# cts198859/deeprl_network

Measured on NVIDIA H100. Metric: agent-env-steps/sec CACC Catch-up NeurComm A2C, higher is better.
Workload: dtype f32

## Files before the change

deeprl_network_b200/csrc/tc_wgrad.cu:

```cuda
#include "bwd_common.cuh"
#include "tc_row.cuh"

extern long long* g_nmarl_prof;

namespace {
using namespace tcrow;

enum { J_GATE0 = 0, J_GATE1, J_ENC_X, J_ENC_M0, J_ENC_M1, J_COUNT };
constexpr int WG_LANES = 128, WG_HALF = 64;
constexpr int WG_A_THREADS = WG_LANES, WG_THREADS = WG_A_THREADS + 2 * 128;
constexpr uint32_t WG_A_TILE = WG_LANES * 128, WG_A_SLOT = 2 * WG_A_TILE;
constexpr uint32_t WG_RING = 224 * 1024;
constexpr int WG_MAX_BARS = 32;
constexpr size_t WG_SMEM = 1024 + WG_RING + WG_MAX_BARS * 8;
static_assert(WG_SMEM <= 232448, "wgrad rings exceed the 227 KB of dynamic shared memory");
static_assert(WG_HALF == ROWS, "each MMA warpgroup covers the 64 rows of one wgmma");
constexpr int WG_REGS_A = 120, WG_REGS_MMA = 192;
static_assert(WG_A_THREADS * WG_REGS_A + 256 * WG_REGS_MMA <= WG_THREADS * 168, "setmaxnreg split exceeds the CTA's registers");
constexpr int SEG_KB = 20;

__device__ __forceinline__ void wg_depths(int N, int& S, int& A) {
  S = N >= 256 ? 2 : (N >= 192 ? 3 : (N >= 128 ? 4 : 6));
  A = (int)((WG_RING - (uint32_t)S * 256u * (uint32_t)N) / WG_A_SLOT);
  if (A > 4) A = 4;
}

struct RingPos {
  int idx = 0; uint32_t ph = 0;
  __device__ __forceinline__ void next(int n) { if (++idx == n) { idx = 0; ph ^= 1u; } }
};

struct TcWgK {
  int B, T, splits, ndp;
  const float* sv_sh; const float* sv_xin; const float* dzT; const float* dpT;
  const float* h_seq; const float* done_pre;
  float* ws;
  long long ws_off[J_COUNT];
  int jobs[J_COUNT]; int n_jobs;
  int* err;
  long long* prof;
};

struct JobDesc {
  const float* A; int F_A, a_feat0, ka_cnt, ones;
  int p_feat0, p_cnt;
  const float* BT; int tile_rows, n_row0, N;
};

__device__ __forceinline__ JobDesc job_desc(const nmarl_model& m, const TcWgK& k, int kind, int i) {
  const nmarl_agent& ag = m.agent[i];
  JobDesc d;
  d.p_feat0 = 0; d.p_cnt = 0;
  const int SD = m.s_dim, LDI = m.kx_pad + m.kp_pad + m.km_pad;
  const int Km = (m.variant == NMARL_IC3) ? NH : ag.n_nbr * NH;
  if (kind == J_GATE0 || kind == J_GATE1) {
    const int mt = kind - J_GATE0;
    d.A = k.sv_sh; d.F_A = SD + NH; d.a_feat0 = 128 * mt; d.ka_cnt = max(0, min(128, SD + NH - 128 * mt)); d.ones = 0;
    d.BT = k.dzT; d.tile_rows = 256; d.n_row0 = 0; d.N = 256;
  } else if (kind == J_ENC_X) {
    d.A = k.sv_xin; d.F_A = LDI; d.a_feat0 = 0; d.ka_cnt = ag.x_nsrc * ag.x_w; d.ones = 1;
    if (m.variant == NMARL_NC) { d.p_feat0 = m.kx_pad; d.p_cnt = ag.n_nbr * m.n_a; }
    d.BT = k.dpT; d.tile_rows = k.ndp; d.n_row0 = 0; d.N = k.ndp;
  } else {
    const int mt = kind - J_ENC_M0;
    d.A = k.sv_xin; d.F_A = LDI; d.a_feat0 = m.kx_pad + m.kp_pad + 128 * mt; d.ka_cnt = max(0, min(128, Km - 128 * mt)); d.ones = 0;
    d.BT = k.dpT; d.tile_rows = k.ndp; d.n_row0 = (m.variant == NMARL_NC) ? 128 : 64; d.N = 64;
  }
  return d;
}

template <bool RAW>
__global__ void __launch_bounds__(WG_THREADS, 1) tc_wgrad_kernel(const __grid_constant__ nmarl_model m,
                                                                 const __grid_constant__ TcWgK k) {
  extern __shared__ uint8_t smem_raw[];
  uint8_t* smem = reinterpret_cast<uint8_t*>((reinterpret_cast<uintptr_t>(smem_raw) + 1023) & ~uintptr_t(1023));

  const int sp = blockIdx.x, jslot = blockIdx.y, i = blockIdx.z;
  const int kind = k.jobs[jslot];
  const JobDesc d = job_desc(m, k, kind, i);
  const int lanes = d.ka_cnt > 0 ? d.ka_cnt + d.ones + d.p_cnt : 0;
  const int nact = (lanes + WG_HALF - 1) / WG_HALF;
  if (nact == 0) return;
  int S, AS;
  wg_depths(d.N, S, AS);
  uint8_t* bst = smem;
  uint8_t* ast = smem + (size_t)S * 256 * d.N;
  uint64_t* bars = reinterpret_cast<uint64_t*>(smem + WG_RING);
  uint64_t *b_full = bars, *b_split = b_full + S, *b_empty = b_split + S, *a_full = b_empty + S, *a_empty = a_full + AS;

  const int N_agents = m.n_agent;
  const int tid = threadIdx.x, warp = tid >> 5;
  const int bpt = k.B / 32;
  const int kb_total = k.T * bpt;
  const int per = (kb_total + k.splits - 1) / k.splits;
  const int kb0 = sp * per, kb1 = min(kb_total, kb0 + per);
  const int nkb = (d.ka_cnt > 0) ? max(0, kb1 - kb0) : 0;
  float* wsj = k.ws + k.ws_off[jslot] + ((size_t)sp * N_agents + i) * 128 * d.N;

  if (tid == 0) {
    for (int s = 0; s < S; ++s) { tc::mbar_init(&b_full[s], 1); tc::mbar_init(&b_split[s], WG_A_THREADS); tc::mbar_init(&b_empty[s], 4 * nact); }
    for (int s = 0; s < AS; ++s) { tc::mbar_init(&a_full[s], WG_A_THREADS); tc::mbar_init(&a_empty[s], 4 * nact); }
    tc::fence_barrier_init();
  }
  __syncthreads();
  const uint32_t tile_bytes = (uint32_t)d.N * 128u;

  if (warp < WG_A_THREADS / 32) {
    asm volatile("setmaxnreg.dec.sync.aligned.u32 %0;" ::"n"(WG_REGS_A));
    const int row = tid;
    const bool on = row < WG_HALF * nact;
    const int ka = row;
    const bool one = d.ones && ka == d.ka_cnt;
    const bool is_p = ka > d.ka_cnt && ka <= d.ka_cnt + d.p_cnt;
    const bool real = on && (ka < d.ka_cnt || is_p);
    const int feat = is_p ? d.p_feat0 + (ka - d.ka_cnt - 1) : d.a_feat0 + ka;
    int hs_agent = -1, hs_unit = 0;
    bool hs_mask = false;
    if (k.h_seq != nullptr && real && !is_p) {
      if ((kind == J_GATE0 || kind == J_GATE1) && feat >= m.s_dim) { hs_agent = i; hs_unit = feat - m.s_dim; hs_mask = true; }
      else if ((kind == J_ENC_M0 || kind == J_ENC_M1) && m.variant == NMARL_NC) {
        const int fm = feat - (m.kx_pad + m.kp_pad);
        hs_agent = m.agent[i].nbr[fm / NH]; hs_unit = fm % NH;
      }
    }
    auto load_x = [&](int q, float (&x)[32]) {
      const int kb = kb0 + q, t = kb / bpt, rb = kb - t * bpt;
      if (hs_agent >= 0) {
        const float* src = k.h_seq + (((size_t)t * N_agents + hs_agent) * NH + hs_unit) * k.B + rb * 32;
#pragma unroll
        for (int p = 0; p < 8; ++p) {
          const float4 v = __ldg(reinterpret_cast<const float4*>(src + 4 * p));
          x[4 * p] = v.x; x[4 * p + 1] = v.y; x[4 * p + 2] = v.z; x[4 * p + 3] = v.w;
        }
        if (hs_mask) {
          const float* dn = k.done_pre + (size_t)t * k.B + rb * 32;
#pragma unroll
          for (int p = 0; p < 8; ++p) {
            const float4 v = __ldg(reinterpret_cast<const float4*>(dn + 4 * p));
            x[4 * p] *= 1.0f - v.x; x[4 * p + 1] *= 1.0f - v.y; x[4 * p + 2] *= 1.0f - v.z; x[4 * p + 3] *= 1.0f - v.w;
          }
        }
      } else if (real) {
        const float* src = d.A + (((size_t)t * N_agents + i) * d.F_A + feat) * k.B + rb * 32;
#pragma unroll
        for (int p = 0; p < 8; ++p) {
          const float4 v = __ldcs(reinterpret_cast<const float4*>(src + 4 * p));
          x[4 * p] = v.x; x[4 * p + 1] = v.y; x[4 * p + 2] = v.z; x[4 * p + 3] = v.w;
        }
      } else {
#pragma unroll
        for (int j = 0; j < 32; ++j) x[j] = one ? 1.0f : 0.0f;
      }
    };
    float xa[32], xb[32];
    RingPos as, bs;
    auto emit_a = [&](int q, float (&x)[32]) {
      tc::mbar_wait(&a_empty[as.idx], as.ph ^ 1, k.err, 11);
      if (on) {
        uint8_t* hi = ast + (size_t)as.idx * WG_A_SLOT;
#pragma unroll
        for (int c = 0; c < 4; ++c) {
          float x8[8];
#pragma unroll
          for (int j = 0; j < 8; ++j) x8[j] = x[8 * c + j];
          tc::st_hilo8(hi, hi + WG_A_TILE, (uint32_t)row, (uint32_t)(8 * c), x8);
        }
        tc::fence_proxy_async();
      }
      tc::mbar_arrive(&a_full[as.idx]);
      as.next(AS);
      if (q + 2 < nkb) load_x(q + 2, x);
      if constexpr (RAW) {
        tc::mbar_wait(&b_full[bs.idx], bs.ph, k.err, 31);
        float4* bhi = reinterpret_cast<float4*>(bst + (size_t)bs.idx * 2 * tile_bytes);
        float4* blo = reinterpret_cast<float4*>(bst + (size_t)bs.idx * 2 * tile_bytes + tile_bytes);
        for (uint32_t e = (uint32_t)tid; e < tile_bytes / 16; e += WG_A_THREADS) {
          const float4 v = bhi[e];
          float4 h, lo4;
          tc::split_tf32(v.x, h.x, lo4.x); tc::split_tf32(v.y, h.y, lo4.y);
          tc::split_tf32(v.z, h.z, lo4.z); tc::split_tf32(v.w, h.w, lo4.w);
          bhi[e] = h;
          blo[e] = lo4;
        }
        tc::fence_proxy_async();
        tc::mbar_arrive(&b_split[bs.idx]);
        bs.next(S);
      }
    };
    if (nkb > 0) load_x(0, xa);
    if (nkb > 1) load_x(1, xb);
    for (int q = 0; q < nkb; q += 2) {
      emit_a(q, xa);
      if (q + 1 < nkb) emit_a(q + 1, xb);
    }
  } else {
    const int g = warp / 4 - 1;
    if (g >= nact) return;
    asm volatile("setmaxnreg.inc.sync.aligned.u32 %0;" ::"n"(WG_REGS_MMA));
    const int t = tid - (g + 1) * 128, w = t >> 5, l = t & 31;
    const bool issuer = g == 0 && t == 0;
    float* out = wsj + g * WG_HALF + 16 * w + (l >> 2);
    long long* prof = (issuer && k.prof != nullptr && sp == 0 && i == 0) ? k.prof + (size_t)jslot * 1024 : nullptr;
    if (prof) { prof[0] = clock64(); prof[3] = kind | (d.N << 8); }
    auto fetch = [&](int q, int st) {
      const int kb = kb0 + q;
      const int tt = kb / bpt, rb = kb - tt * bpt;
      const size_t pair = (size_t)(2 * d.tile_rows * 128);
      const size_t off = RAW ? (size_t)tt * N_agents * bpt * pair + ((size_t)i * bpt + rb) * (pair / 2)
                             : (((size_t)tt * N_agents + i) * bpt + rb) * pair;
      const uint8_t* tile = reinterpret_cast<const uint8_t*>(d.BT) + off;
      uint8_t* dst = bst + (size_t)st * 2 * tile_bytes;
      tc::mbar_arrive_expect_tx(&b_full[st], RAW ? tile_bytes : 2 * tile_bytes);
      tc::bulk_g2s(dst, tile + (size_t)d.n_row0 * 128, tile_bytes, &b_full[st]);
      if (!RAW) tc::bulk_g2s(dst + tile_bytes, tile + (size_t)(d.tile_rows + d.n_row0) * 128, tile_bytes, &b_full[st]);
    };
    if (issuer)
      for (int q = 0; q < S && q < nkb; ++q) fetch(q, q);
    float acc[128];
#pragma unroll
    for (int j = 0; j < 128; ++j) acc[j] = 0.f;
    auto drain = [&](bool rmw) {
#pragma unroll
      for (int j = 0; j < 32; ++j) {
        if (8 * j < d.N) {
          const int n = 8 * j + 2 * (l & 3);
#pragma unroll
          for (int e = 0; e < 4; ++e) {
            float* o = out + (size_t)(n + (e & 1)) * 128 + 8 * (e >> 1);
            *o = rmw ? *o + acc[4 * j + e] : acc[4 * j + e];
          }
        }
      }
    };
    RingPos as, bs;
    for (int q = 0; q < nkb; ++q) {
      const bool seg_first = (q % SEG_KB) == 0;
      uint8_t* b = bst + (size_t)bs.idx * 2 * tile_bytes;
      if constexpr (RAW) tc::mbar_wait(&b_split[bs.idx], bs.ph, k.err, 33);
      else tc::mbar_wait(&b_full[bs.idx], bs.ph, k.err, 31);
      if (prof && q < 300) prof[4 + 3 * q] = clock64();
      tc::mbar_wait(&a_full[as.idx], as.ph, k.err, 32);
      if (prof && q < 300) prof[5 + 3 * q] = clock64();
      uint8_t* a = ast + (size_t)as.idx * WG_A_SLOT + g * (WG_A_TILE / 2);
      tc::wgmma_fence();
      tc::wgmma_kblock_3x(d.N, acc, tc::smem_desc_sw128(a), tc::smem_desc_sw128(a + WG_A_TILE), tc::smem_desc_sw128(b),
                          tc::smem_desc_sw128(b + tile_bytes), 4, seg_first);
      tc::wgmma_commit();
      tc::wgmma_wait_all();
      if (prof && q < 300) prof[6 + 3 * q] = clock64();
      if (l == 0) { tc::mbar_arrive(&a_empty[as.idx]); tc::mbar_arrive(&b_empty[bs.idx]); }
      if (issuer && q + S < nkb) {
        tc::mbar_wait(&b_empty[bs.idx], bs.ph, k.err, 34);
        fetch(q + S, bs.idx);
      }
      as.next(AS); bs.next(S);
      if ((q + 1) % SEG_KB == 0 || q + 1 == nkb) drain(q >= SEG_KB);
    }
    if (nkb == 0) drain(false);
    if (prof) { prof[1] = min(nkb, 300); prof[2] = clock64(); }
  }
}

__global__ void __launch_bounds__(256) tc_wgrad_reduce_kernel(const __grid_constant__ nmarl_model m, const __grid_constant__ TcWgK k,
                                                             float* __restrict__ grads) {
  const int jslot = blockIdx.y, i = blockIdx.z, kind = k.jobs[jslot];
  const JobDesc d = job_desc(m, k, kind, i);
  const nmarl_agent& ag = m.agent[i];
  const int lanes = d.ka_cnt + (d.ones ? 1 : 0) + d.p_cnt;
  const int total = 128 * d.N;
  for (int e = blockIdx.x * blockDim.x + threadIdx.x; e < total; e += gridDim.x * blockDim.x) {
    const int ln = e & 127, n = e >> 7;
    if (ln >= lanes) continue;
    float s = 0.f;
    for (int sp = 0; sp < k.splits; ++sp) s += k.ws[k.ws_off[jslot] + (((size_t)sp * m.n_agent + i) * d.N + n) * 128 + ln];
    if (kind == J_GATE0 || kind == J_GATE1) grads[ag.o_wxh + (size_t)(128 * (kind - J_GATE0) + ln) * NG + n] = s;
    else if (kind == J_ENC_X) {
      if (ln < d.ka_cnt) { if (n < NH) grads[ag.o_w_ob + ln * NH + n] = s; }
      else if (ln > d.ka_cnt) { if (n >= NH && n < 2 * NH) grads[ag.o_w_fp + (ln - d.ka_cnt - 1) * NH + n - NH] = s; }
      else if (n < NH) grads[ag.o_b_ob + n] = s;
      else if (m.variant == NMARL_NC && n < 2 * NH) grads[ag.o_b_fp + n - NH] = s;
      else if (ag.o_b_msg >= 0) grads[ag.o_b_msg + n - ((m.variant == NMARL_NC) ? 2 * NH : NH)] = s;
    } else grads[ag.o_w_msg + (size_t)(128 * (kind - J_ENC_M0) + ln) * NH + n] = s;
  }
}

__global__ void __launch_bounds__(256) gate_bias_reduce_kernel(const __grid_constant__ nmarl_model m, const float* __restrict__ part,
                                                              int tiles, int T, float* __restrict__ grads) {
  __shared__ float red[8][32];
  const int c = threadIdx.x & 31, p = threadIdx.x >> 5, col = blockIdx.x * 32 + c, i = blockIdx.y;
  const int n = T * tiles;
  float s = 0.f;
  for (int e = p; e < n; e += 8) {
    const int t = e / tiles, tile = e - t * tiles;
    s += part[(((size_t)t * m.n_agent + i) * tiles + tile) * NG + col];
  }
  red[p][c] = s;
  __syncthreads();
  if (p == 0) {
    float tsum = 0.f;
    for (int w = 0; w < 8; ++w) tsum += red[w][c];
    grads[m.agent[i].o_b + col] = tsum;
  }
}

NMARL_PARAMS_FIT(nmarl_model, TcWgK);
NMARL_PARAMS_FIT(nmarl_model, TcWgK, float*);
NMARL_PARAMS_FIT(nmarl_model, const float*, int, int, float*);

int job_list(const nmarl_model* m, int* jobs) {
  int n = 0;
  jobs[n++] = J_GATE0;
  if (m->s_dim + NH > 128) jobs[n++] = J_GATE1;
  jobs[n++] = J_ENC_X;
  if (m->variant != NMARL_IA2C) {
    jobs[n++] = J_ENC_M0;
    if (m->km_pad > 128) jobs[n++] = J_ENC_M1;
  }
  return n;
}
int job_N(const nmarl_model* m, int kind) {
  if (kind == J_GATE0 || kind == J_GATE1) return 256;
  if (kind == J_ENC_X) return nmarl_tc_ndp(m);
  return 64;
}

}

int nmarl_tc_ndp(const nmarl_model* m) { return m->variant == NMARL_NC ? 192 : (m->variant == NMARL_IA2C ? 64 : 128); }

int nmarl_tc_wgrad_splits(int n_agent) {
  int s = 33;
  while (4 * s * n_agent > 132 * 8 && s > 1) s = (s + 1) / 2;
  return s;
}

int64_t nmarl_tc_wgrad_ws_floats(const nmarl_model* m) {
  int jobs[J_COUNT];
  const int nj = job_list(m, jobs);
  int64_t tot = 0;
  for (int j = 0; j < nj; ++j) tot += (int64_t)nmarl_tc_wgrad_splits(m->n_agent) * m->n_agent * 128 * job_N(m, jobs[j]);
  return tot;
}

int nmarl_tc_launch_wgrads(const nmarl_model* m, int B, int T, const float* sv_sh, const float* sv_xin, const float* dzT,
                           const float* dpT, const float* sv_dz, float* ws, float* grads, int* err, cudaStream_t st,
                           cudaStream_t st_bias, bool raw_tiles, void** ev_wgrad, const float* h_seq, const float* done_pre) {
  TcWgK k{};
  k.B = B; k.T = T; k.splits = nmarl_tc_wgrad_splits(m->n_agent); k.ndp = nmarl_tc_ndp(m);
  k.sv_sh = sv_sh; k.sv_xin = sv_xin; k.dzT = dzT; k.dpT = dpT; k.ws = ws; k.err = err;
  k.h_seq = h_seq; k.done_pre = done_pre; k.prof = g_nmarl_prof;
  k.n_jobs = job_list(m, k.jobs);
  long long off = 0;
  for (int j = 0; j < k.n_jobs; ++j) { k.ws_off[j] = off; off += (long long)k.splits * m->n_agent * 128 * job_N(m, k.jobs[j]); }
  static bool configured = false;
  if (!configured) {
    NMARL_CUDA(cudaFuncSetAttribute(tc_wgrad_kernel<false>, cudaFuncAttributeMaxDynamicSharedMemorySize, (int)WG_SMEM));
    NMARL_CUDA(cudaFuncSetAttribute(tc_wgrad_kernel<true>, cudaFuncAttributeMaxDynamicSharedMemorySize, (int)WG_SMEM));
    configured = true;
  }
  gate_bias_reduce_kernel<<<dim3(NG / 32, m->n_agent), 256, 0, st_bias>>>(*m, sv_dz, B / 32, T, grads);
  NMARL_LAUNCH_CHECK();
  if (ev_wgrad) NMARL_CUDA(cudaEventRecord((cudaEvent_t)ev_wgrad[0], st));
  const dim3 grid(k.splits, k.n_jobs, m->n_agent);
  if (raw_tiles) tc_wgrad_kernel<true><<<grid, WG_THREADS, WG_SMEM, st>>>(*m, k);
  else tc_wgrad_kernel<false><<<grid, WG_THREADS, WG_SMEM, st>>>(*m, k);
  NMARL_LAUNCH_CHECK();
  if (ev_wgrad) NMARL_CUDA(cudaEventRecord((cudaEvent_t)ev_wgrad[1], st));
  NMARL_DBG_SYNC(st, "tc_wgrad_kernel");
  tc_wgrad_reduce_kernel<<<dim3(64, k.n_jobs, m->n_agent), 256, 0, st>>>(*m, k, grads);
  NMARL_LAUNCH_CHECK();
  NMARL_DBG_SYNC(st, "tc_wgrad_reduce");
  return 0;
}
```

Measured before the change: 52.87 million.

## Stage wgrad A-operand loads through cp.async landing buffers and specialize MMA loop on N

The A-producer warps now prefetch their activation rows with cp.async into a swizzled, double-buffered shared-memory landing zone one k-block ahead. The done mask also goes through this path. This replaces the register-held two-deep ldg pipeline and the emit_a lambda. The MMA consumer loop is templated on N (64/128/192/256) so the wgmma k-block and the drain are compile-time unrolled. Ring depths are retuned: N=192 now uses 2 B stages, and the A depth is reduced to make room for the landing buffers. The split and A-store ordering is also merged under one fence. Together this is meant to free producer registers and hide global latency, at the cost of extra shared memory and fewer A/B ring stages.

```diff
diff --git a/deeprl_network_b200/csrc/tc_wgrad.cu b/deeprl_network_b200/csrc/tc_wgrad.cu
--- a/deeprl_network_b200/csrc/tc_wgrad.cu
+++ b/deeprl_network_b200/csrc/tc_wgrad.cu
@@ -1,5 +1,6 @@
 #include "bwd_common.cuh"
 #include "tc_row.cuh"
+#include <type_traits>
 
 extern long long* g_nmarl_prof;
 
@@ -12,7 +13,8 @@
 constexpr uint32_t WG_A_TILE = WG_LANES * 128, WG_A_SLOT = 2 * WG_A_TILE;
 constexpr uint32_t WG_RING = 224 * 1024;
 constexpr int WG_MAX_BARS = 32;
-constexpr size_t WG_SMEM = 1024 + WG_RING + WG_MAX_BARS * 8;
+constexpr uint32_t WG_LAND = WG_LANES * 128;
+constexpr size_t WG_SMEM = 1024 + WG_RING + WG_MAX_BARS * 8 + 4 * 2 * 128;
 static_assert(WG_SMEM <= 232448, "wgrad rings exceed the 227 KB of dynamic shared memory");
 static_assert(WG_HALF == ROWS, "each MMA warpgroup covers the 64 rows of one wgmma");
 constexpr int WG_REGS_A = 120, WG_REGS_MMA = 192;
@@ -20,10 +22,17 @@
 constexpr int SEG_KB = 20;
 
 __device__ __forceinline__ void wg_depths(int N, int& S, int& A) {
-  S = N >= 256 ? 2 : (N >= 192 ? 3 : (N >= 128 ? 4 : 6));
-  A = (int)((WG_RING - (uint32_t)S * 256u * (uint32_t)N) / WG_A_SLOT);
+  S = N >= 192 ? 2 : (N >= 128 ? 4 : 6);
+  A = (int)((WG_RING - (uint32_t)S * 256u * (uint32_t)N - 2 * WG_LAND) / WG_A_SLOT);
   if (A > 4) A = 4;
 }
+
+__device__ __forceinline__ void cp_async16(void* smem_dst, const void* gsrc) {
+  asm volatile("cp.async.cg.shared.global [%0], [%1], 16;" ::"r"(tc::smem_u32(smem_dst)), "l"(gsrc) : "memory");
+}
+__device__ __forceinline__ void cp_async_commit() { asm volatile("cp.async.commit_group;" ::: "memory"); }
+template <int N>
+__device__ __forceinline__ void cp_async_wait() { asm volatile("cp.async.wait_group %0;" ::"n"(N) : "memory"); }
 
 struct RingPos {
   int idx = 0; uint32_t ph = 0;
@@ -123,57 +132,59 @@
         hs_agent = m.agent[i].nbr[fm / NH]; hs_unit = fm % NH;
       }
     }
-    auto load_x = [&](int q, float (&x)[32]) {
-      const int kb = kb0 + q, t = kb / bpt, rb = kb - t * bpt;
-      if (hs_agent >= 0) {
-        const float* src = k.h_seq + (((size_t)t * N_agents + hs_agent) * NH + hs_unit) * k.B + rb * 32;
-#pragma unroll
-        for (int p = 0; p < 8; ++p) {
-          const float4 v = __ldg(reinterpret_cast<const float4*>(src + 4 * p));
-          x[4 * p] = v.x; x[4 * p + 1] = v.y; x[4 * p + 2] = v.z; x[4 * p + 3] = v.w;
+    const bool gate_hs = k.h_seq != nullptr && (kind == J_GATE0 || kind == J_GATE1);
+    const int lane = tid & 31;
+    uint8_t* land = ast + (size_t)AS * WG_A_SLOT;
+    float* dn_sm = reinterpret_cast<float*>(smem + WG_RING + WG_MAX_BARS * 8) + warp * 2 * 32;
+    auto issue = [&](int q) {
+      if (q < nkb) {
+        const int kb = kb0 + q, t = kb / bpt, rb = kb - t * bpt;
+        const float* src = hs_agent >= 0 ? k.h_seq + (((size_t)t * N_agents + hs_agent) * NH + hs_unit) * k.B + rb * 32
+                         : real ? d.A + (((size_t)t * N_agents + i) * d.F_A + feat) * k.B + rb * 32 : nullptr;
+        if (src != nullptr) {
+          uint8_t* dst = land + (size_t)(q & 1) * WG_LAND + (size_t)row * 128;
+#pragma unroll
+          for (int c = 0; c < 8; ++c) cp_async16(dst + (((c ^ row) & 7) << 4), src + 4 * c);
+        }
+        if (gate_hs) {
+          __syncwarp();
+          if (lane < 8) cp_async16(dn_sm + (q & 1) * 32 + 4 * lane, k.done_pre + (size_t)t * k.B + rb * 32 + 4 * lane);
+        }
+      }
+      cp_async_commit();
+    };
+    auto read_x = [&](int q, float (&x)[32]) {
+      cp_async_wait<1>();
+      if (gate_hs) __syncwarp();
+      if (hs_agent >= 0 || real) {
+        const uint8_t* src = land + (size_t)(q & 1) * WG_LAND + (size_t)row * 128;
+#pragma unroll
+        for (int c = 0; c < 8; ++c) {
+          const float4 v = *reinterpret_cast<const float4*>(src + (((c ^ row) & 7) << 4));
+          x[4 * c] = v.x; x[4 * c + 1] = v.y; x[4 * c + 2] = v.z; x[4 * c + 3] = v.w;
         }
         if (hs_mask) {
-          const float* dn = k.done_pre + (size_t)t * k.B + rb * 32;
+          const float4* dn = reinterpret_cast<const float4*>(dn_sm + (q & 1) * 32);
 #pragma unroll
           for (int p = 0; p < 8; ++p) {
-            const float4 v = __ldg(reinterpret_cast<const float4*>(dn + 4 * p));
+            const float4 v = dn[p];
             x[4 * p] *= 1.0f - v.x; x[4 * p + 1] *= 1.0f - v.y; x[4 * p + 2] *= 1.0f - v.z; x[4 * p + 3] *= 1.0f - v.w;
           }
         }
-      } else if (real) {
-        const float* src = d.A + (((size_t)t * N_agents + i) * d.F_A + feat) * k.B + rb * 32;
-#pragma unroll
-        for (int p = 0; p < 8; ++p) {
-          const float4 v = __ldcs(reinterpret_cast<const float4*>(src + 4 * p));
-          x[4 * p] = v.x; x[4 * p + 1] = v.y; x[4 * p + 2] = v.z; x[4 * p + 3] = v.w;
-        }
       } else {
 #pragma unroll
         for (int j = 0; j < 32; ++j) x[j] = one ? 1.0f : 0.0f;
       }
     };
-    float xa[32], xb[32];
     RingPos as, bs;
-    auto emit_a = [&](int q, float (&x)[32]) {
-      tc::mbar_wait(&a_empty[as.idx], as.ph ^ 1, k.err, 11);
-      if (on) {
-        uint8_t* hi = ast + (size_t)as.idx * WG_A_SLOT;
-#pragma unroll
-        for (int c = 0; c < 4; ++c) {
-          float x8[8];
-#pragma unroll
-          for (int j = 0; j < 8; ++j) x8[j] = x[8 * c + j];
-          tc::st_hilo8(hi, hi + WG_A_TILE, (uint32_t)row, (uint32_t)(8 * c), x8);
-        }
-        tc::fence_proxy_async();
-      }
-      tc::mbar_arrive(&a_full[as.idx]);
-      as.next(AS);
-      if (q + 2 < nkb) load_x(q + 2, x);
+    issue(0);
+    for (int q = 0; q < nkb; ++q) {
+      issue(q + 1);
       if constexpr (RAW) {
         tc::mbar_wait(&b_full[bs.idx], bs.ph, k.err, 31);
         float4* bhi = reinterpret_cast<float4*>(bst + (size_t)bs.idx * 2 * tile_bytes);
         float4* blo = reinterpret_cast<float4*>(bst + (size_t)bs.idx * 2 * tile_bytes + tile_bytes);
+#pragma unroll 2
         for (uint32_t e = (uint32_t)tid; e < tile_bytes / 16; e += WG_A_THREADS) {
           const float4 v = bhi[e];
           float4 h, lo4;
@@ -182,16 +193,24 @@
           bhi[e] = h;
           blo[e] = lo4;
         }
-        tc::fence_proxy_async();
-        tc::mbar_arrive(&b_split[bs.idx]);
-        bs.next(S);
-      }
-    };
-    if (nkb > 0) load_x(0, xa);
-    if (nkb > 1) load_x(1, xb);
-    for (int q = 0; q < nkb; q += 2) {
-      emit_a(q, xa);
-      if (q + 1 < nkb) emit_a(q + 1, xb);
+      }
+      float x[32];
+      read_x(q, x);
+      tc::mbar_wait(&a_empty[as.idx], as.ph ^ 1, k.err, 11);
+      if (on) {
+        uint8_t* hi = ast + (size_t)as.idx * WG_A_SLOT;
+#pragma unroll
+        for (int c = 0; c < 4; ++c) {
+          float x8[8];
+#pragma unroll
+          for (int j = 0; j < 8; ++j) x8[j] = x[8 * c + j];
+          tc::st_hilo8(hi, hi + WG_A_TILE, (uint32_t)row, (uint32_t)(8 * c), x8);
+        }
+      }
+      tc::fence_proxy_async();
+      if constexpr (RAW) { tc::mbar_arrive(&b_split[bs.idx]); bs.next(S); }
+      tc::mbar_arrive(&a_full[as.idx]);
+      as.next(AS);
     }
   } else {
     const int g = warp / 4 - 1;
@@ -219,10 +238,11 @@
     float acc[128];
 #pragma unroll
     for (int j = 0; j < 128; ++j) acc[j] = 0.f;
-    auto drain = [&](bool rmw) {
-#pragma unroll
-      for (int j = 0; j < 32; ++j) {
-        if (8 * j < d.N) {
+    auto run = [&](auto n_c) {
+      constexpr int N = decltype(n_c)::value;
+      auto drain = [&](bool rmw) {
+#pragma unroll
+        for (int j = 0; j < N / 8; ++j) {
           const int n = 8 * j + 2 * (l & 3);
 #pragma unroll
           for (int e = 0; e < 4; ++e) {
@@ -230,33 +250,39 @@
             *o = rmw ? *o + acc[4 * j + e] : acc[4 * j + e];
           }
         }
-      }
+      };
+      RingPos as, bs;
+      for (int q = 0; q < nkb; ++q) {
+        const bool seg_first = (q % SEG_KB) == 0;
+        uint8_t* b = bst + (size_t)bs.idx * 2 * tile_bytes;
+        if constexpr (RAW) tc::mbar_wait(&b_split[bs.idx], bs.ph, k.err, 33);
+        else tc::mbar_wait(&b_full[bs.idx], bs.ph, k.err, 31);
+        if (prof && q < 300) prof[4 + 3 * q] = clock64();
+        tc::mbar_wait(&a_full[as.idx], as.ph, k.err, 32);
+        if (prof && q < 300) prof[5 + 3 * q] = clock64();
+        uint8_t* a = ast + (size_t)as.idx * WG_A_SLOT + g * (WG_A_TILE / 2);
+        tc::wgmma_fence();
+        tc::wgmma_kblock_3x<N, 4>(acc, tc::smem_desc_sw128(a), tc::smem_desc_sw128(a + WG_A_TILE), tc::smem_desc_sw128(b),
+                                  tc::smem_desc_sw128(b + tile_bytes), seg_first);
+        tc::wgmma_commit();
+        tc::wgmma_wait_all();
+        if (prof && q < 300) prof[6 + 3 * q] = clock64();
+        if (l == 0) { tc::mbar_arrive(&a_empty[as.idx]); tc::mbar_arrive(&b_empty[bs.idx]); }
+        if (issuer && q + S < nkb) {
+          tc::mbar_wait(&b_empty[bs.idx], bs.ph, k.err, 34);
+          fetch(q + S, bs.idx);
+        }
+        as.next(AS); bs.next(S);
+        if ((q + 1) % SEG_KB == 0 || q + 1 == nkb) drain(q >= SEG_KB);
+      }
+      if (nkb == 0) drain(false);
     };
-    RingPos as, bs;
-    for (int q = 0; q < nkb; ++q) {
-      const bool seg_first = (q % SEG_KB) == 0;
-      uint8_t* b = bst + (size_t)bs.idx * 2 * tile_bytes;
-      if constexpr (RAW) tc::mbar_wait(&b_split[bs.idx], bs.ph, k.err, 33);
-      else tc::mbar_wait(&b_full[bs.idx], bs.ph, k.err, 31);
-      if (prof && q < 300) prof[4 + 3 * q] = clock64();
-      tc::mbar_wait(&a_full[as.idx], as.ph, k.err, 32);
-      if (prof && q < 300) prof[5 + 3 * q] = clock64();
-      uint8_t* a = ast + (size_t)as.idx * WG_A_SLOT + g * (WG_A_TILE / 2);
-      tc::wgmma_fence();
-      tc::wgmma_kblock_3x(d.N, acc, tc::smem_desc_sw128(a), tc::smem_desc_sw128(a + WG_A_TILE), tc::smem_desc_sw128(b),
-                          tc::smem_desc_sw128(b + tile_bytes), 4, seg_first);
-      tc::wgmma_commit();
-      tc::wgmma_wait_all();
-      if (prof && q < 300) prof[6 + 3 * q] = clock64();
-      if (l == 0) { tc::mbar_arrive(&a_empty[as.idx]); tc::mbar_arrive(&b_empty[bs.idx]); }
-      if (issuer && q + S < nkb) {
-        tc::mbar_wait(&b_empty[bs.idx], bs.ph, k.err, 34);
-        fetch(q + S, bs.idx);
-      }
-      as.next(AS); bs.next(S);
-      if ((q + 1) % SEG_KB == 0 || q + 1 == nkb) drain(q >= SEG_KB);
+    switch (d.N) {
+      case 64: run(std::integral_constant<int, 64>{}); break;
+      case 128: run(std::integral_constant<int, 128>{}); break;
+      case 192: run(std::integral_constant<int, 192>{}); break;
+      default: run(std::integral_constant<int, 256>{}); break;
     }
-    if (nkb == 0) drain(false);
     if (prof) { prof[1] = min(nkb, 300); prof[2] = clock64(); }
   }
 }
```

Measured after the change: 53.85 million (median of 6 runs). 1.02x the previous value.

## Share TF32 B-tile split with MMA warps and specialize wgrad on N

Applied to the files above, without the earlier changes.

The hi/lo TF32 split of each raw B tile is now done by the A-producer threads together with the MMA warpgroups, with the split barrier count raised to match. The MMA loop is templated on N via a compile-time switch, so accumulator arrays and the drain loop are sized exactly and the wgmma call takes N as a template argument. Ring positions are derived from q instead of RingPos counters, and per-stage profiling stamps are extended. The aim is to take the split off the critical path of the 128 producer threads and to cut register and branch overhead in the MMA loop. In exchange, the MMA warps spend time on the split, and the extra template instantiations grow code size.

```diff
diff --git a/deeprl_network_b200/csrc/tc_wgrad.cu b/deeprl_network_b200/csrc/tc_wgrad.cu
--- a/deeprl_network_b200/csrc/tc_wgrad.cu
+++ b/deeprl_network_b200/csrc/tc_wgrad.cu
@@ -1,6 +1,7 @@
 #include "bwd_common.cuh"
 #include "tc_row.cuh"
 
+#include <type_traits>
 extern long long* g_nmarl_prof;
 
 namespace {
@@ -40,6 +41,19 @@
   int* err;
   long long* prof;
 };
+
+enum { PS_B_READY, PS_A_READY, PS_RETIRED, PS_LANDED, PS_SPLIT, PS_LOADED, PS_A_FILLED, PROF_KB };
+constexpr int PROF_STRIDE = 2048, PROF_MAX_KB = (PROF_STRIDE - 4) / PROF_KB;
+__device__ __forceinline__ void stamp(long long* prof, int q, int what) {
+  if (prof != nullptr && q < PROF_MAX_KB) prof[4 + PROF_KB * q + what] = clock64();
+}
+__device__ __forceinline__ void stamp_after(long long* prof, int q, int what, float v) {
+  if (prof == nullptr || q >= PROF_MAX_KB) return;
+  long long c;
+  asm volatile("{\n\t.reg .pred p;\n\tsetp.lt.f32 p, %1, 0f00000000;\n\tmov.u64 %0, %%clock64;\n\t@p add.s64 %0, %0, 1;\n\t}"
+               : "=l"(c) : "f"(v) : "memory");
+  prof[4 + PROF_KB * q + what] = c;
+}
 
 struct JobDesc {
   const float* A; int F_A, a_feat0, ka_cnt, ones;
@@ -97,8 +111,9 @@
   const int nkb = (d.ka_cnt > 0) ? max(0, kb1 - kb0) : 0;
   float* wsj = k.ws + k.ws_off[jslot] + ((size_t)sp * N_agents + i) * 128 * d.N;
 
+  const int split_threads = WG_A_THREADS + 128 * nact;
   if (tid == 0) {
-    for (int s = 0; s < S; ++s) { tc::mbar_init(&b_full[s], 1); tc::mbar_init(&b_split[s], WG_A_THREADS); tc::mbar_init(&b_empty[s], 4 * nact); }
+    for (int s = 0; s < S; ++s) { tc::mbar_init(&b_full[s], 1); tc::mbar_init(&b_split[s], split_threads); tc::mbar_init(&b_empty[s], 4 * nact); }
     for (int s = 0; s < AS; ++s) { tc::mbar_init(&a_full[s], WG_A_THREADS); tc::mbar_init(&a_empty[s], 4 * nact); }
     tc::fence_barrier_init();
   }
@@ -154,8 +169,10 @@
     };
     float xa[32], xb[32];
     RingPos as, bs;
+    long long* prof = (tid == 0 && k.prof != nullptr && sp == 0 && i == 0) ? k.prof + (size_t)jslot * PROF_STRIDE : nullptr;
     auto emit_a = [&](int q, float (&x)[32]) {
       tc::mbar_wait(&a_empty[as.idx], as.ph ^ 1, k.err, 11);
+      stamp_after(prof, q, PS_LOADED, x[31]);
       if (on) {
         uint8_t* hi = ast + (size_t)as.idx * WG_A_SLOT;
 #pragma unroll
@@ -168,13 +185,16 @@
         tc::fence_proxy_async();
       }
       tc::mbar_arrive(&a_full[as.idx]);
+      stamp(prof, q, PS_A_FILLED);
       as.next(AS);
       if (q + 2 < nkb) load_x(q + 2, x);
       if constexpr (RAW) {
         tc::mbar_wait(&b_full[bs.idx], bs.ph, k.err, 31);
+        stamp(prof, q, PS_LANDED);
         float4* bhi = reinterpret_cast<float4*>(bst + (size_t)bs.idx * 2 * tile_bytes);
         float4* blo = reinterpret_cast<float4*>(bst + (size_t)bs.idx * 2 * tile_bytes + tile_bytes);
-        for (uint32_t e = (uint32_t)tid; e < tile_bytes / 16; e += WG_A_THREADS) {
+#pragma unroll 4
+        for (uint32_t e = (uint32_t)tid; e < tile_bytes / 16; e += split_threads) {
           const float4 v = bhi[e];
           float4 h, lo4;
           tc::split_tf32(v.x, h.x, lo4.x); tc::split_tf32(v.y, h.y, lo4.y);
@@ -183,6 +203,7 @@
           blo[e] = lo4;
         }
         tc::fence_proxy_async();
+        stamp(prof, q, PS_SPLIT);
         tc::mbar_arrive(&b_split[bs.idx]);
         bs.next(S);
       }
@@ -200,7 +221,7 @@
     const int t = tid - (g + 1) * 128, w = t >> 5, l = t & 31;
     const bool issuer = g == 0 && t == 0;
     float* out = wsj + g * WG_HALF + 16 * w + (l >> 2);
-    long long* prof = (issuer && k.prof != nullptr && sp == 0 && i == 0) ? k.prof + (size_t)jslot * 1024 : nullptr;
+    long long* prof = (issuer && k.prof != nullptr && sp == 0 && i == 0) ? k.prof + (size_t)jslot * PROF_STRIDE : nullptr;
     if (prof) { prof[0] = clock64(); prof[3] = kind | (d.N << 8); }
     auto fetch = [&](int q, int st) {
       const int kb = kb0 + q;
@@ -216,13 +237,14 @@
     };
     if (issuer)
       for (int q = 0; q < S && q < nkb; ++q) fetch(q, q);
-    float acc[128];
-#pragma unroll
-    for (int j = 0; j < 128; ++j) acc[j] = 0.f;
-    auto drain = [&](bool rmw) {
-#pragma unroll
-      for (int j = 0; j < 32; ++j) {
-        if (8 * j < d.N) {
+    auto run = [&](auto n_tag) {
+      constexpr int N = decltype(n_tag)::value;
+      float acc[N / 2];
+#pragma unroll
+      for (int j = 0; j < N / 2; ++j) acc[j] = 0.f;
+      auto drain = [&](bool rmw) {
+#pragma unroll
+        for (int j = 0; j < N / 8; ++j) {
           const int n = 8 * j + 2 * (l & 3);
 #pragma unroll
           for (int e = 0; e < 4; ++e) {
@@ -230,34 +252,66 @@
             *o = rmw ? *o + acc[4 * j + e] : acc[4 * j + e];
           }
         }
+      };
+      auto issue = [&](int q, bool first) {
+        const int st = q % S, slot = q % AS;
+        if constexpr (RAW) {
+          {
+            tc::mbar_wait(&b_full[st], (q / S) & 1, k.err, 31);
+            float4* bhi = reinterpret_cast<float4*>(bst + (size_t)st * 2 * tile_bytes);
+            float4* blo = reinterpret_cast<float4*>(bst + (size_t)st * 2 * tile_bytes + tile_bytes);
+#pragma unroll 2
+            for (uint32_t e = (uint32_t)tid; e < tile_bytes / 16; e += split_threads) {
+              const float4 v = bhi[e];
+              float4 h, lo4;
+              tc::split_tf32(v.x, h.x, lo4.x); tc::split_tf32(v.y, h.y, lo4.y);
+              tc::split_tf32(v.z, h.z, lo4.z); tc::split_tf32(v.w, h.w, lo4.w);
+              bhi[e] = h;
+              blo[e] = lo4;
+            }
+            tc::fence_proxy_async();
+            tc::mbar_arrive(&b_split[st]);
+          }
+          tc::mbar_wait(&b_split[st], (q / S) & 1, k.err, 33);
+        }
+        else tc::mbar_wait(&b_full[st], (q / S) & 1, k.err, 31);
+        stamp(prof, q, PS_B_READY);
+        tc::mbar_wait(&a_full[slot], (q / AS) & 1, k.err, 32);
+        stamp(prof, q, PS_A_READY);
+        const uint8_t* a = ast + (size_t)slot * WG_A_SLOT + g * (WG_A_TILE / 2);
+        const uint8_t* b = bst + (size_t)st * 2 * tile_bytes;
+        tc::wgmma_fence();
+        tc::wgmma_kblock_3x<N, 4>(acc, tc::smem_desc_sw128(a), tc::smem_desc_sw128(a + WG_A_TILE), tc::smem_desc_sw128(b),
+                                  tc::smem_desc_sw128(b + tile_bytes), first);
+        tc::wgmma_commit();
+      };
+      auto release = [&](int q) {
+        stamp(prof, q, PS_RETIRED);
+        const int st = q % S;
+        if (l == 0) { tc::mbar_arrive(&a_empty[q % AS]); tc::mbar_arrive(&b_empty[st]); }
+        if (issuer && q + S < nkb) {
+          tc::mbar_wait(&b_empty[st], (q / S) & 1, k.err, 34);
+          fetch(q + S, st);
+        }
+      };
+      for (int q0 = 0; q0 < nkb; q0 += SEG_KB) {
+        const int qe = min(nkb, q0 + SEG_KB) - 1;
+        for (int q = q0; q <= qe; ++q) {
+          issue(q, q == q0);
+          tc::wgmma_wait<0>();
+          release(q);
+        }
+        drain(q0 > 0);
       }
+      if (nkb == 0) drain(false);
     };
-    RingPos as, bs;
-    for (int q = 0; q < nkb; ++q) {
-      const bool seg_first = (q % SEG_KB) == 0;
-      uint8_t* b = bst + (size_t)bs.idx * 2 * tile_bytes;
-      if constexpr (RAW) tc::mbar_wait(&b_split[bs.idx], bs.ph, k.err, 33);
-      else tc::mbar_wait(&b_full[bs.idx], bs.ph, k.err, 31);
-      if (prof && q < 300) prof[4 + 3 * q] = clock64();
-      tc::mbar_wait(&a_full[as.idx], as.ph, k.err, 32);
-      if (prof && q < 300) prof[5 + 3 * q] = clock64();
-      uint8_t* a = ast + (size_t)as.idx * WG_A_SLOT + g * (WG_A_TILE / 2);
-      tc::wgmma_fence();
-      tc::wgmma_kblock_3x(d.N, acc, tc::smem_desc_sw128(a), tc::smem_desc_sw128(a + WG_A_TILE), tc::smem_desc_sw128(b),
-                          tc::smem_desc_sw128(b + tile_bytes), 4, seg_first);
-      tc::wgmma_commit();
-      tc::wgmma_wait_all();
-      if (prof && q < 300) prof[6 + 3 * q] = clock64();
-      if (l == 0) { tc::mbar_arrive(&a_empty[as.idx]); tc::mbar_arrive(&b_empty[bs.idx]); }
-      if (issuer && q + S < nkb) {
-        tc::mbar_wait(&b_empty[bs.idx], bs.ph, k.err, 34);
-        fetch(q + S, bs.idx);
-      }
-      as.next(AS); bs.next(S);
-      if ((q + 1) % SEG_KB == 0 || q + 1 == nkb) drain(q >= SEG_KB);
+    switch (d.N) {
+      case 64: run(std::integral_constant<int, 64>{}); break;
+      case 128: run(std::integral_constant<int, 128>{}); break;
+      case 192: run(std::integral_constant<int, 192>{}); break;
+      default: run(std::integral_constant<int, 256>{}); break;
     }
-    if (nkb == 0) drain(false);
-    if (prof) { prof[1] = min(nkb, 300); prof[2] = clock64(); }
+    if (prof) { prof[1] = min(nkb, PROF_MAX_KB); prof[2] = clock64(); }
   }
 }
 
```

Result: no change. 52.85 million before, 52.97 million after, median of 6 (+0.2%).
